# ZHANGKEON/DIS-YOLO

Measured on AMD Instinct MI355X. Metric: train images/sec @576x576 bf16, higher is better.
Workload: dtype bf16

## Files before the change

### dis-yolo_amd/csrc/conv_wgrad.hip

```cpp
#include "common.h"
#include "runtime.h"

namespace {

struct WgradParams {
  const bf16* x0;
  const bf16* x1;
  const bf16* dy;
  float* out;
  int B, H, W, C0, C1, Cin;
  int Ho, Wo, Cout, ldy;
  int ks, stride, pad_t, pad_l;
  int M, K;
  int steps_per_split, steps;
  int tilesK, tilesN;
  unsigned bytes0, bytes1, bytesy;
};

typedef __attribute__((address_space(3))) s16x4 lds_s16x4;
typedef int i32x4 __attribute__((ext_vector_type(4)));
constexpr unsigned OOB = 0x80000000u;

__device__ __forceinline__ int swz_u(int row, int u, int units) {
  const int h = (row & 3) | (((row >> 3) & 1) << 2);
// ... 461 lines not shown
  }

  float* slab = p.out + (size_t)bsplit * 9 * p.Cin * p.Cout;
  wait_vmcnt<0>();
  __syncthreads();
  constexpr int WTN = CO_T / 2;
  constexpr int ROWP = WTN * 4 + 16;
  constexpr int CPR4 = WTN / 4;
  char* sw = smem + wave * (16 * ROWP);
#pragma unroll
  for (int i = 0; i < TPW; ++i) {
    if (NW == 8 && i >= ntaps) continue;
    const int tap = tap0 + i;
#pragma unroll
    for (int j = 0; j < NJ; ++j)
#pragma unroll
      for (int r = 0; r < 4; ++r) *reinterpret_cast<float*>(sw + (g * 4 + r) * ROWP + (j * 16 + li) * 4) = acc[i][j][r];
    __builtin_amdgcn_fence(__ATOMIC_RELEASE, "wavefront");
    __builtin_amdgcn_wave_barrier();
    __builtin_amdgcn_fence(__ATOMIC_ACQUIRE, "wavefront");
#pragma unroll
    for (int it = 0; it < (16 * CPR4) / 64; ++it) {
      const int idx = it * 64 + lane;
      const int row = idx / CPR4, c4 = idx % CPR4;
      const int kk = tap * p.Cin + ci0 + u * 16 + row, n = co0 + ch * WTN + c4 * 4;
      if (n < p.Cout && !(p.debug & 1))
        *reinterpret_cast<float4*>(slab + (size_t)kk * p.Cout + n) = *reinterpret_cast<const float4*>(sw + row * ROWP + c4 * 16);
    }
    __builtin_amdgcn_fence(__ATOMIC_RELEASE, "wavefront");
    __builtin_amdgcn_wave_barrier();
  }
}

__global__ __launch_bounds__(256) void slab_reduce_kernel(const float* slabs, float* out, int64_t n, int splits) {
  __shared__ float sh[4][64];
  const int o = threadIdx.x & 63, g = threadIdx.x >> 6;
  const int64_t i = (int64_t)blockIdx.x * 64 + o;
  float a0 = 0.f, a1 = 0.f, a2 = 0.f, a3 = 0.f;
  if (i < n) {
    int k = g;
    for (; k + 12 < splits; k += 16) {
      a0 += slabs[(size_t)k * n + i];
      a1 += slabs[(size_t)(k + 4) * n + i];
      a2 += slabs[(size_t)(k + 8) * n + i];
      a3 += slabs[(size_t)(k + 12) * n + i];
    }
    for (; k < splits; k += 4) a0 += slabs[(size_t)k * n + i];
  }
  sh[g][o] = (a0 + a1) + (a2 + a3);
  __syncthreads();
  if (g == 0 && i < n) out[i] = (sh[0][o] + sh[1][o]) + (sh[2][o] + sh[3][o]);
}

__global__ __launch_bounds__(1024) void conv_first_wgrad_kernel(const float* img, const bf16* dy, float* slabs, int B,
                                                                int H, int W, int Cout, int px_per_block) {
  const int M = B * H * W;
  const int o = threadIdx.x;
  const int nout = 27 * Cout;
  if (o >= nout) return;
  const int k = o / Cout, co = o - k * Cout;
  const int tap = k / 3, ci = k - tap * 3;
  const int kh = tap / 3, kw = tap - kh * 3;
  const int m0 = blockIdx.x * px_per_block;
  int m1 = m0 + px_per_block;
  if (m1 > M) m1 = M;
  float acc = 0.f;
  for (int m = m0; m < m1; ++m) {
    const int b = m / (H * W);
    const int rem = m - b * H * W;
    const int y = rem / W, x = rem - y * W;
    const int iy = y + kh - 1, ix = x + kw - 1;
    if ((unsigned)iy < (unsigned)H && (unsigned)ix < (unsigned)W)
      acc += img[((size_t)(b * H + iy) * W + ix) * 3 + ci] * (float)dy[(size_t)m * Cout + co];
  }
  slabs[(size_t)blockIdx.x * nout + o] = acc;
}

constexpr int F1_ROWB = 272;
constexpr int F1_IMGB = 27 * F1_ROWB + 80;
constexpr int F1_STB = F1_IMGB + 8192;

__global__ __launch_bounds__(512) void conv_first_wgrad_mfma_kernel(const float* img, const bf16* dy, float* slabs, int B,
                                                                   int H, int W, int units_x, int nunits, unsigned bytesy) {
  extern __shared__ __attribute__((aligned(16))) char smem[];
// ... 273 lines not shown
  if (plan3(d, opts, &q3)) {
    Wg3Params p;
    p.x = (const bf16*)d->x0;
    p.dy = (const bf16*)dy;
    p.B = d->B; p.H = d->H; p.W = d->W; p.Cin = d->C0; p.Cout = d->Cout; p.ldy = dy_ld;
    p.Ho = d->Ho; p.Wo = d->Wo;
    p.P = d->Wo + 1; p.Hp = d->Ho + 1; p.frame = p.Hp * p.P;
    p.kbias = q3.s2 ? 0 : ceil_div((q3.leadB + 1) * 64, p.frame);
    p.a64 = 64 / p.P; p.r64 = 64 % p.P;
    p.chunks = q3.chunks; p.chunks_per_split = q3.cps;
    p.tilesCi = q3.tilesCi; p.tilesCo = q3.tilesCo; p.tiles = q3.tilesCi * q3.tilesCo;
    p.leadA = q3.leadA; p.leadB = q3.leadB;
    p.bytesx = (unsigned)((size_t)d->B * d->H * d->W * d->C0 * 2);
    p.bytesy = (unsigned)((size_t)d->B * d->Ho * d->Wo * dy_ld * 2);
    p.out = q3.splits == 1 ? dw : (float*)workspace;
    p.debug = 0;
    hipStream_t s = (hipStream_t)stream;
    if (opts & DISYOLO_WGRAD_REDUCE_ONLY) goto reduce3;
    if (q3.s2) {
      launch3_s2(p, q3, s);
    } else if (q3.co_t == 128) {
      if (q3.R == 8) launch3<128, 8>(p, q3, s);
      else if (q3.R == 16) launch3<128, 16>(p, q3, s);
      else launch3<128, 32>(p, q3, s);
    } else {
      if (q3.R == 8) launch3<64, 8>(p, q3, s);
      else if (q3.R == 16) launch3<64, 16>(p, q3, s);
      else launch3<64, 32>(p, q3, s);
    }
    DY_CHECK_LAUNCH();
  reduce3:
    if (q3.splits > 1 && !(opts & DISYOLO_WGRAD_PARTIAL_ONLY)) {
      const int64_t n = (int64_t)9 * p.Cin * p.Cout;
      hipLaunchKernelGGL(slab_reduce_kernel, dim3(ceil_div(n, 64)), dim3(256), 0, s, (const float*)workspace, dw, n,
                         q3.splits);
      DY_CHECK_LAUNCH();
    }
    return DISYOLO_OK;
  }
  WgradParams p;
  p.x0 = (const bf16*)d->x0;
  p.x1 = (const bf16*)d->x1;
  p.dy = (const bf16*)dy;
  p.B = d->B; p.H = d->H; p.W = d->W; p.C0 = d->C0; p.C1 = d->C1; p.Cin = d->C0 + d->C1;
  p.Ho = d->Ho; p.Wo = d->Wo; p.Cout = d->Cout; p.ldy = dy_ld;
  p.ks = d->ksize; p.stride = d->stride; p.pad_t = d->pad_t; p.pad_l = d->pad_l;
  p.M = d->B * d->Ho * d->Wo;
  p.K = d->ksize * d->ksize * p.Cin;
  p.bytes0 = (unsigned)((size_t)d->B * d->H * d->W * d->C0 * 2);
  p.bytes1 = (unsigned)((size_t)d->B * (d->H / 2) * (d->W / 2) * d->C1 * 2);
  p.bytesy = (unsigned)((size_t)p.M * dy_ld * 2);
  int bn, splits;
  plan(d, &bn, &splits, &p.steps_per_split, &p.steps);
  p.out = splits == 1 ? dw : (float*)workspace;
  hipStream_t s = (hipStream_t)stream;
  p.tilesK = ceil_div(p.K, 128);
  p.tilesN = ceil_div(p.Cout, bn);
  dim3 grid(p.tilesK * p.tilesN * splits);
  const int sto = (opts & DISYOLO_WGRAD_STAGES_MASK) >> 4;
  const int st = sto ? sto + 1 : 3;
  if (opts & DISYOLO_WGRAD_REDUCE_ONLY) goto reduce1;
#define DY_WG(BNV, YB)                                                                                   \
  if (st == 2) hipLaunchKernelGGL((conv_wgrad_kernel<BNV, 2>), grid, dim3(256), 2 * (8192 + YB), s, p);      \
  else if (st == 3) hipLaunchKernelGGL((conv_wgrad_kernel<BNV, 3>), grid, dim3(256), 3 * (8192 + YB), s, p); \
  else hipLaunchKernelGGL((conv_wgrad_kernel<BNV, 4>), grid, dim3(256), 4 * (8192 + YB), s, p);
  if (bn == 128) { DY_WG(128, 8192) }
  else if (bn == 64) { DY_WG(64, 4096) }
  else { DY_WG(32, 4096) }
#undef DY_WG
  DY_CHECK_LAUNCH();
reduce1:
  if (splits > 1 && !(opts & DISYOLO_WGRAD_PARTIAL_ONLY)) {
    const int64_t n = (int64_t)p.K * p.Cout;
    hipLaunchKernelGGL(slab_reduce_kernel, dim3(ceil_div(n, 64)), dim3(256), 0, s, (const float*)workspace, dw, n,
                       splits);
    DY_CHECK_LAUNCH();
  }
  return DISYOLO_OK;
}

static int first_wgrad_blocks(int B, int H, int W) {
  const int64_t pairs = ((int64_t)B * H * ceil_div(W, 128) + 1) / 2;
  return (int)(pairs < 512 ? pairs : 512);
}

extern "C" size_t disyolo_conv_first_wgrad_workspace(int B, int H, int W, int Cout) {
  const int64_t M = (int64_t)B * H * W;
  const int blocks = ceil_div(M, 1024);
  const size_t direct = (size_t)blocks * 27 * Cout * sizeof(float);
  const size_t mfma = (size_t)first_wgrad_blocks(B, H, W) * 27 * 32 * sizeof(float);
  return direct > mfma ? direct : mfma;
}

extern "C" int disyolo_conv_first_wgrad(const float* images, const void* dy, float* dw, int B, int H, int W, int Cout,
                                        void* workspace, size_t workspace_bytes, void* stream) {
  DY_REQUIRE(images && dy && dw && B > 0 && H > 0 && W > 0 && Cout > 0 && 27 * Cout <= 1024, "first_wgrad: bad args");
  if (!workspace || workspace_bytes < disyolo_conv_first_wgrad_workspace(B, H, W, Cout)) {
    disyolo_set_error("first_wgrad: workspace too small");
    return DISYOLO_E_WORKSPACE;
  }
  DY_RECORD_OR_RUN([=](void* s) { return disyolo_conv_first_wgrad(images, dy, dw, B, H, W, Cout, workspace, workspace_bytes, s); });
  const int64_t M = (int64_t)B * H * W;
  hipStream_t s = (hipStream_t)stream;
  const int64_t n = 27 * Cout;
  if (Cout == 32 && M * 64 < (1LL << 31)) {
    const int units_x = ceil_div(W, 128);
    const int nunits = B * H * units_x;
    const int blocks = first_wgrad_blocks(B, H, W);
    hipLaunchKernelGGL(conv_first_wgrad_mfma_kernel, dim3(blocks), dim3(512), 4 * F1_STB, s, images, (const bf16*)dy,
                       (float*)workspace, B, H, W, units_x, nunits, (unsigned)(M * 64));
    DY_CHECK_LAUNCH();
    hipLaunchKernelGGL(slab_reduce_kernel, dim3(ceil_div(n, 64)), dim3(256), 0, s, (const float*)workspace, dw, n, blocks);
    DY_CHECK_LAUNCH();
    return DISYOLO_OK;
  }
  const int blocks = ceil_div(M, 1024);
  hipLaunchKernelGGL(conv_first_wgrad_kernel, dim3(blocks), dim3(1024), 0, s, images, (const bf16*)dy,
                     (float*)workspace, B, H, W, Cout, 1024);
  DY_CHECK_LAUNCH();
  hipLaunchKernelGGL(slab_reduce_kernel, dim3(ceil_div(n, 64)), dim3(256), 0, s, (const float*)workspace, dw, n,
                     blocks);
  DY_CHECK_LAUNCH();
  return DISYOLO_OK;
}
```

### dis-yolo_amd/lib.py

```python
from __future__ import annotations

import ctypes as C
import os
from typing import Optional

import numpy as np
import torch

_HERE = os.path.dirname(os.path.abspath(__file__))
LIB_PATH = os.environ.get("DISYOLO_LIB", os.path.join(_HERE, "libdisyolo_hip.so"))

GRAD_LD = 32
ROI_MAX = 16
ROI_W = 12
K_MAPS = (3, 5, 7)
MASK_STRIDES = (1, 2, 4)


def roi_w(k: int) -> int:
    return 2 * (k + 1) + 4


def block32_post(k: int) -> int:
    return {3: 1, 5: 2, 7: 3}[k]
# ... 29 lines not shown
_SIGS = {
    "disyolo_version": (C.c_int, []),
    "disyolo_last_error": (C.c_char_p, []),
    "disyolo_conv_desc_size": (C.c_size_t, []),
    "disyolo_find_contours": (C.c_int, [C.c_void_p, C.c_int, C.c_int, C.c_void_p, C.c_int64, C.c_void_p, C.c_void_p, C.c_int,
                                        C.POINTER(C.c_int), C.POINTER(C.c_int64)]),
    "disyolo_conv2d_stats_rows": (C.c_int, [C.POINTER(ConvDesc)]),
    "disyolo_conv2d_bn_bwd_stats_ok": (C.c_int, [C.POINTER(ConvDesc)]),
    "disyolo_conv2d_bn_fused_ok": (C.c_int, [C.POINTER(ConvDesc)]),
    "disyolo_cluster_sync_words": (C.c_int, [C.c_int]),
    "disyolo_cluster_sync_error": (C.c_int, [C.c_void_p, C.c_int]),
    "disyolo_conv2d_fwd": (C.c_int, [C.POINTER(ConvDesc), C.c_void_p]),
    "disyolo_conv2d_tile": (C.c_int, [C.POINTER(ConvDesc)] + [C.POINTER(C.c_int)] * 4),
    "disyolo_conv_first_fwd": (C.c_int, [C.c_void_p] * 5 + [C.c_int] * 4 + [C.c_float, C.c_void_p]),
    "disyolo_conv12_fused_ok": (C.c_int, [C.c_int] * 3),
    "disyolo_conv12_fused_fwd": (C.c_int, [C.c_void_p] * 8 + [C.c_int] * 3 + [C.c_float, C.c_void_p]),
    "disyolo_block32_fused_ok": (C.c_int, [C.c_int] * 6),
    "disyolo_block64_fused_ok": (C.c_int, [C.c_int] * 4),
    "disyolo_pack_quad": (C.c_int, [C.c_void_p, C.c_void_p, C.c_int, C.c_int, C.c_void_p]),
    "disyolo_dgrad_s2_quad_ok": (C.c_int, [C.c_int] * 5),
    "disyolo_dgrad_s2_quad": (C.c_int, [C.c_void_p] * 4 + [C.c_int] * 5 + [C.c_void_p]),
    "disyolo_block64_fused_fwd": (C.c_int, [C.c_void_p] * 8 + [C.c_int] * 4 + [C.c_float, C.c_void_p]),
    "disyolo_block32_fused_fwd": (C.c_int, [C.c_void_p, C.c_void_p, C.c_int, C.c_int] + [C.c_void_p] * 6 + [C.c_int] +
                                  [C.c_void_p] * 3 + [C.c_int] * 3 + [C.c_float, C.c_void_p]),
    "disyolo_conv2d_wgrad_workspace": (C.c_size_t, [C.POINTER(ConvDesc), C.c_int]),
    "disyolo_conv2d_wgrad": (C.c_int, [C.POINTER(ConvDesc), C.c_void_p, C.c_int, C.c_void_p, C.c_void_p,
                                       C.c_size_t, C.c_int, C.c_void_p]),
    "disyolo_conv2d_fp8_fwd": (C.c_int, [C.POINTER(ConvDesc), C.c_void_p, C.c_void_p, C.c_void_p, C.c_void_p, C.c_float,
                                         C.c_void_p, C.c_float, C.c_void_p, C.c_void_p]),
    "disyolo_conv_first_fwd_fp8": (C.c_int, [C.c_void_p] * 5 + [C.c_float] + [C.c_int] * 4 + [C.c_float, C.c_void_p]),
    "disyolo_quant_fp8": (C.c_int, [C.c_void_p, C.c_int, C.c_void_p, C.c_int64, C.c_float, C.c_void_p]),
    "disyolo_dequant_fp8": (C.c_int, [C.c_void_p, C.c_void_p, C.c_int64, C.c_float, C.c_void_p]),
    "disyolo_pack_weights_fp8": (C.c_int, [C.c_void_p, C.c_void_p] + [C.c_int] * 3 + [C.c_float, C.c_void_p]),
    "disyolo_conv2d_wgrad_plan": (C.c_int, [C.POINTER(ConvDesc), C.c_int] + [C.POINTER(C.c_int)] * 4),
    "disyolo_conv_first_wgrad_workspace": (C.c_size_t, [C.c_int] * 4),
    "disyolo_conv_first_wgrad": (C.c_int, [C.c_void_p] * 3 + [C.c_int] * 4 + [C.c_void_p, C.c_size_t, C.c_void_p]),
    "disyolo_image_pad8": (C.c_int, [C.c_void_p, C.c_void_p, C.c_int64, C.c_void_p]),
    "disyolo_copy2d_f32": (C.c_int, [C.c_void_p, C.c_void_p] + [C.c_int] * 4 + [C.c_void_p]),
    "disyolo_pack_weights": (C.c_int, [C.c_void_p] * 3 + [C.c_int] * 4 + [C.c_void_p]),
    "disyolo_pack_table_bytes": (C.c_size_t, [C.c_int]),
    "disyolo_pack_table_build": (C.c_int, [C.c_void_p, C.c_int, C.c_void_p, C.POINTER(C.c_int)]),
    "disyolo_pack_all": (C.c_int, [C.c_void_p, C.c_int, C.c_int, C.c_void_p]),
    "disyolo_bn_finalize": (C.c_int, [C.c_void_p, C.c_int, C.c_int, C.c_int64] + [C.c_void_p] * 4 +
                            [C.c_float, C.c_float] + [C.c_void_p] * 5),
    "disyolo_colstats_rows": (C.c_int, [C.c_int64, C.c_int]),
    "disyolo_colstats": (C.c_int, [C.c_void_p, C.c_void_p, C.c_int64, C.c_int, C.c_void_p]),
    "disyolo_bn_fold": (C.c_int, [C.c_void_p] * 4 + [C.c_float] + [C.c_void_p] * 2 + [C.c_int, C.c_void_p]),
    "disyolo_bn_act_fwd": (C.c_int, [C.c_void_p] * 5 + [C.c_int64, C.c_int, C.c_float, C.c_void_p]),
    "disyolo_bn_act_bwd_workspace": (C.c_size_t, [C.c_int64, C.c_int]),
    "disyolo_bn_act_bwd_partials_workspace": (C.c_size_t, [C.c_int]),
    "disyolo_bn_act_bwd_partials": (C.c_int, [C.c_void_p] * 9 + [C.c_int64, C.c_int, C.c_float, C.c_void_p, C.c_int,
                                              C.c_void_p, C.c_int, C.c_void_p, C.c_size_t, C.c_void_p]),
    "disyolo_bn_partial_sums": (C.c_int, [C.c_void_p, C.c_int, C.c_int, C.c_void_p, C.c_void_p]),
    "disyolo_bn_finalize_sums": (C.c_int, [C.c_void_p, C.c_int, C.c_int64] + [C.c_void_p] * 4 + [C.c_float, C.c_float] +
                                 [C.c_void_p] * 5),
    "disyolo_bn_bwd_reduce_rows": (C.c_int, [C.c_int64, C.c_int]),
    "disyolo_bn_bwd_reduce": (C.c_int, [C.c_void_p] * 6 + [C.c_int64, C.c_int, C.c_float, C.c_void_p, C.c_void_p, C.c_size_t,
                                        C.c_void_p]),
    "disyolo_bn_bwd_apply_sums": (C.c_int, [C.c_void_p] * 8 + [C.c_int64] + [C.c_void_p] * 3 + [C.c_int64, C.c_int, C.c_float,
                                            C.c_void_p, C.c_int, C.c_void_p, C.c_size_t, C.c_void_p]),
    "disyolo_bn_act_bwd": (C.c_int, [C.c_void_p] * 9 + [C.c_int64, C.c_int, C.c_float, C.c_void_p, C.c_int, C.c_void_p, C.c_size_t,
                                                       C.c_void_p]),
    "disyolo_upsample2x_bwd": (C.c_int, [C.c_void_p] * 2 + [C.c_int] * 7 + [C.c_void_p]),
    "disyolo_colsum_workspace": (C.c_size_t, [C.c_int64, C.c_int]),
    "disyolo_colsum": (C.c_int, [C.c_void_p, C.c_void_p, C.c_int64, C.c_int, C.c_int, C.c_void_p, C.c_size_t,
                                 C.c_void_p]),
# ... 102 lines not shown
    return None if t is None else t.data_ptr()


def _stream() -> int:
    return torch.cuda.current_stream().cuda_stream


def _need(t: torch.Tensor, dtype, name: str) -> None:
    if t.dtype != dtype or not t.is_cuda or not t.is_contiguous():
        raise DisyoloError("%s must be a contiguous CUDA tensor of %s (got %s on %s)" % (name, dtype, t.dtype, t.device))


def _need_shape(t: torch.Tensor, shape, name: str) -> None:
    if tuple(t.shape) != tuple(shape):
        raise DisyoloError("%s must have shape %s (got %s)" % (name, tuple(shape), tuple(t.shape)))


class Workspace:

    def __init__(self, device):
        self.device = device
        self.buf = torch.empty(1 << 20, dtype=torch.uint8, device=device)
        self.frozen = False

    def get(self, nbytes: int) -> torch.Tensor:
        if self.buf.numel() < nbytes:
            if self.frozen:
                raise DisyoloError("workspace of %d bytes is frozen by a recorded command list; %d requested"
                                   % (self.buf.numel(), nbytes))
            self.buf = torch.empty(int(nbytes * 1.25) + 256, dtype=torch.uint8, device=self.device)
        return self.buf


class CmdList:

    def __init__(self):
        self.h = load().disyolo_cmdlist_create()
        self.keep = []
        self._side = None
        self._lanes = {}

    def __del__(self):
        try:
            if self.h:
                if torch.cuda.is_available() and (self._side is not None or self._lanes):
                    for st in [self._side] + list(self._lanes.values()):
                        if st is not None:
                            torch.cuda.current_stream(st.device).wait_stream(st)
                load().disyolo_cmdlist_destroy(self.h)
        except Exception:
            pass

    def __enter__(self):
        global TIMER
        if TIMER is not None:
            raise DisyoloError("cannot record a command list while the kernel timer is active")
        _check(load().disyolo_cmdlist_begin(self.h), "cmdlist_begin")
        global CURRENT_LANE
        CURRENT_LANE = 0
        return self

    def __exit__(self, *exc):
        _check(load().disyolo_cmdlist_end(), "cmdlist_end")
        global CURRENT_LANE
        CURRENT_LANE = 0
        return False
# ... 359 lines not shown
        TIMER.run("block64_kernel", 2.0 * M * (64 * 128 + 128 * 576), fn, float(M * 512))
        return
    fn()


def conv_first_fwd(images, w_hwio, scale, shift, y, alpha=0.1) -> None:
    _need(images, torch.float32, "images")
    _need(y, torch.bfloat16, "y")
    B, H, W, _ = images.shape
    _check(load().disyolo_conv_first_fwd(_p(images), _p(w_hwio), _p(scale), _p(shift), _p(y), B, H, W, y.shape[-1],
                                         alpha, _stream()), "conv_first_fwd")


WGRAD_IM2COL, WGRAD_PARTIAL_ONLY, WGRAD_REDUCE_ONLY = 1, 2, 4


def wgrad_stages(n: int) -> int:
    if not 2 <= int(n) <= 4:
        raise DisyoloError("wgrad_stages: 2..4 pipeline stages (got %r)" % (n,))
    return (int(n) - 1) << 4


def conv2d_wgrad_workspace(d: ConvDesc, opts: int = 0) -> int:
    return load().disyolo_conv2d_wgrad_workspace(C.byref(d), opts)


def conv2d_wgrad(d: ConvDesc, dy, dy_ld: int, dw, ws: Workspace, opts: int = 0) -> None:
    need = conv2d_wgrad_workspace(d, opts)
    buf = ws.get(need)

    def call(o):
        _check(load().disyolo_conv2d_wgrad(C.byref(d), _p(dy), dy_ld, _p(dw), _p(buf), buf.numel(), o, _stream()),
               "conv2d_wgrad")
    if TIMER is not None and not (opts & (WGRAD_PARTIAL_ONLY | WGRAD_REDUCE_ONLY)):
        kind, tn, ring, splits = conv2d_wgrad_plan(d, opts)
        name = ("conv_wgrad3x3_kernel<%d,%d,3,4,0>" % (tn, ring)) if kind == 1 else ("conv_wgrad_kernel<%d,3>" % tn)
        if kind == 1 and d.stride == 2:
            name = "conv_wgrad3x3_kernel<64,8,3,4,1>"
        TIMER.run(name, conv_flops(d), lambda: call(opts | WGRAD_PARTIAL_ONLY))
        if splits > 1:
            TIMER.run("slab_reduce_kernel", 0.0, lambda: call(opts | WGRAD_REDUCE_ONLY))
        return
    call(opts)


def conv2d_wgrad_plan(d: ConvDesc, opts: int = 0):
    v = [C.c_int(0) for _ in range(4)]
    _check(load().disyolo_conv2d_wgrad_plan(C.byref(d), opts, *[C.byref(x) for x in v]), "conv2d_wgrad_plan")
    return tuple(x.value for x in v)


def conv_first_wgrad(images, dy, dw, ws: Workspace) -> None:
    B, H, W, _ = images.shape
    cout = dy.shape[-1]
    need = load().disyolo_conv_first_wgrad_workspace(B, H, W, cout)
    buf = ws.get(need)
    _check(load().disyolo_conv_first_wgrad(_p(images), _p(dy), _p(dw), B, H, W, cout, _p(buf), buf.numel(), _stream()),
           "conv_first_wgrad")


def copy2d_f32(src, dst, rows, cols, src_ld, dst_ld) -> None:
    _check(load().disyolo_copy2d_f32(_p(src), _p(dst), rows, cols, src_ld, dst_ld, _stream()), "copy2d_f32")


def pack_weights(w_hwio, w_fwd, w_dgrad, ksize, cin, cout, cout_pad=0) -> None:
    _check(load().disyolo_pack_weights(_p(w_hwio), _p(w_fwd), _p(w_dgrad), ksize, cin, cout, max(cout_pad, cout),
                                       _stream()), "pack_weights")


class PackJob(C.Structure):
    _fields_ = [("w_hwio", C.c_void_p), ("w_fwd", C.c_void_p), ("w_dgrad", C.c_void_p),
                ("ksize", C.c_int32), ("Cin", C.c_int32), ("Cout", C.c_int32), ("cout_pad", C.c_int32)]


class PackTable:

    def __init__(self, jobs, device):
        n = len(jobs)
        arr = (PackJob * n)()
        for i, (w, wf, wd, k, cin, cout, pad) in enumerate(jobs):
            arr[i] = PackJob(_p(w), _p(wf), _p(wd), k, cin, cout, pad)
        nbytes = load().disyolo_pack_table_bytes(n)
# ... 397 lines not shown
```

### dis-yolo_amd/net.py

```python
from __future__ import annotations

from typing import Dict, List, Optional, Sequence, Tuple

import math
import json
import contextlib
import os
import sys
import numpy as np
import torch

from . import config as cfg
from . import lib as L

BF16 = torch.bfloat16
F32 = torch.float32

WGRAD_GROUP = 3
OPT_CHUNK_ELEMS = 8_000_000
PIPE_LANE = 2


class Layer:
    __slots__ = ("idx", "cin", "cout", "k", "stride", "kind", "src", "src_up", "shortcut", "lock", "H", "W", "Ho",
# ... 366 lines not shown
            g1 = S // 32
            self.labels = [torch.zeros(B, g, g, 3, 5 + self.num_class, dtype=F32, device=dev)
                           for g in (4 * g1, 2 * g1, g1)]
            self.true_boxes = torch.zeros(B, G, 5, dtype=F32, device=dev)
            self.true_masks = torch.zeros(B, G, S, S, dtype=torch.uint8, device=dev)
            self.perm_det = torch.arange(cfg.MAX_DETECTION, dtype=torch.int32, device=dev).repeat(B, 1).contiguous()
            self.perm_gt = torch.arange(G, dtype=torch.int32, device=dev).repeat(B, 1).contiguous()
            self.rois = torch.zeros(B, L.ROI_MAX, L.roi_w(self.k), dtype=torch.int32, device=dev)
            self.roi_count = torch.zeros(B, dtype=torch.int32, device=dev)
            self._in_sets = None
            if self.pair:
                names = ("labels", "true_boxes", "true_masks", "perm_det", "perm_gt", "clip_window")
                first = {n: getattr(self, n) for n in names}
                second = {n: ([t.clone() for t in v] if isinstance(v, list) else v.clone()) for n, v in first.items()}
                self._in_sets = [first, second]
            self.losses = torch.zeros(8, dtype=F32, device=dev)
            self.mask_loss = torch.zeros(1, dtype=F32, device=dev)
            self.reg_loss = torch.zeros(1, dtype=F32, device=dev)
            self.loss_ring = torch.zeros(self.LOSS_RING, dtype=F32, device=dev)
            tmax = 0
            for l in self.layers:
                if l.src_up is not None and l.wdg is not None:
                    tmax = max(tmax, B * l.H * l.W * self.by_idx[l.src_up].cout)
            self.up_tmp = torch.zeros(max(tmax, 1), dtype=BF16, device=dev)
            need = 1 << 20
            for l in self.layers:
                if l.wgrad_desc is not None:
                    need = max(need, L.conv2d_wgrad_workspace(l.wgrad_desc))
                if l.dx is not None and l.kind != "lin":
                    need = max(need, L.load().disyolo_bn_act_bwd_workspace(B * l.Ho * l.Wo, l.cout))
            if not l1.lock:
                need = max(need, L.load().disyolo_conv_first_wgrad_workspace(B, S, S, l1.cout))
            self.ws.get(int(need))
            self.ws_aux.get(int(need))
        self.ws_det.get(int(max(L.load().disyolo_detect_workspace(B, S, self.num_class), 1 << 20)))
        self._build_dgrad_descs()
        self.refresh_weights()

    FP8_FROM = int(os.environ.get("DISYOLO_FP8_FROM", "10"))
    FP8_UPTO = 52
    FP8_DUAL = (4, 9, 26, 43, 52)

    def _fp8_layers(self):
        return [l for l in self.layers if self.FP8_FROM <= l.idx <= self.FP8_UPTO and (l.lock or not self.training)]

    def _plan_fp8(self) -> None:
        dev = self.device
        ls = self._fp8_layers()
        if [l.idx for l in ls] != list(range(self.FP8_FROM, self.FP8_UPTO + 1)) or not all(
                l.lock or not self.training for l in self.layers[:self.FP8_UPTO]):
            raise L.DisyoloError("dtype='fp8' needs conv1-52 in inference mode (stage 1 training, or training=False)")
        if self.FP8_FROM <= 1 and any(1 in (l.src, l.src_up) for l in self.layers if l.idx > 2):
            raise L.DisyoloError("dtype='fp8' with DISYOLO_FP8_FROM=1 and mask_stride=1: conv83 needs act1 in bf16")
        self._fp8_entry = self.by_idx[self.FP8_FROM - 1] if self.FP8_FROM > 1 else None
        if self._fp8_entry is not None:
            q = self._fp8_entry
            q.act8 = torch.zeros(self.B, q.Ho, q.Wo, q.cout, dtype=torch.uint8, device=dev)
            q.s_out = 1.0
        for l in ls:
            l.act8 = torch.zeros(self.B, l.Ho, l.Wo, l.cout, dtype=torch.uint8, device=dev)
            l.escale = torch.zeros(l.cout, dtype=F32, device=dev)
            l.dual16 = l.idx in self.FP8_DUAL
            l.s_out, l.s_w = 1.0, 1.0
            if l.idx > 1:
                l.w8 = torch.zeros(l.cout, l.k * l.k * l.cin, dtype=torch.uint8, device=dev)
                l.desc8 = L.make_conv_desc(self.by_idx[l.src].act8, l.w8, l.act8, l.k, l.stride, leaky=True, alpha=cfg.ALPHA)

# ... 681 lines not shown
                                 bn_bwd=(tgt.raw, tgt.scale, tgt.shift, tgt.mean, tgt.rstd, tgt.bwd_part, cfg.ALPHA),
                                 bn_bwd_fused=dict(dgamma=tgt.dgamma, dbeta=tgt.dbeta, sync=tgt.csync_bwd))
            tgt.fused_bwd = True
        L.conv2d_fwd(d)

    def check_cluster_sync(self) -> None:
        for l in self.layers:
            for name, buf in (("forward", l.csync), ("backward", l.csync_bwd)):
                if buf is not None:
                    code = L.cluster_sync_error(buf, l.cout)
                    if code:
                        raise L.DisyoloError("conv%d: the in-launch batch-norm exchange (%s) timed out (code %#x): another launch of "
                                             "that kind was running on this device, or the grid was not resident; the results of "
                                             "this run are wrong (DISYOLO_BN_INKERNEL=0 switches the feature off)" % (l.idx, name, code))

    def _shortcut_feeds_grad(self, tgt: Layer) -> bool:
        return tgt.shortcut is not None and self.by_idx[tgt.shortcut].grad is not None

    def _final_writers(self, visit) -> Dict[int, Tuple[int, str]]:
        last: Dict[int, Tuple[int, str]] = {}
        for l in visit:
            if l.lock:
                continue
            if l.kind != "lin" and l.shortcut is not None and self.by_idx[l.shortcut].grad is not None:
                last[l.shortcut] = (l.idx, "add")
            for mode, tgt, _ in l.dgrad_descs:
                last[tgt.idx] = (l.idx, mode)
        return last

    def backward_order(self) -> List[Layer]:
        heads = [self.by_idx[i] for i in (75, 74, 67, 66, 59, 58)]
        return heads + [l for l in reversed(self.layers) if l.idx not in self.HEAD_LAYERS]

    def backward(self, on_layer_done=None, sweep: bool = False) -> None:
        B = self.B
        for l in self.layers:
            l.grad_set = False
        visit = self.backward_order()
        order = [l for l in visit if not l.lock]
        final_of = {} if self.sync_bn else self._final_writers(visit)
        for l in self.layers:
            l.bwd_part_rows = 0
            l.fused_bwd = False
        inl = self.dp is not None and self.dp.inlist
        overlap_opt = sweep and (self.dp is None or inl) and self.n_params > 0
        if overlap_opt:
            if self.opt_chunks is None:
                self._plan_opt_chunks()
            self._opt_swept = set()
            self._opt_done = [set() for _ in self.opt_chunks]
        pending: list = []

        def flush():
            if not pending:
                return
            side_g = pending[0][4]
            mark = L.lane_mark(0) if side_g else None
            waited = False
            for (pl, pdx, pld, pM, pside) in pending:
                if pside:
                    if not waited:
                        L.lane_wait(mark, 1)
                        waited = True
                    L.set_lane(1)
                wsl = self.ws_aux if pside else self.ws
                if pl.kind == "lin":
                    L.colsum(pl.dx, pl.dbias, pM, pl.cout_pad, pl.cout, wsl)
                if pl.idx == 1:
                    L.conv_first_wgrad(self.images, pl.dx, pl.dw, wsl)
                else:
                    L.conv2d_wgrad(pl.wgrad_desc, pdx, pld, pl.dw, wsl)
                if pside:
                    L.set_lane(0)
                if self._overlap_rec:
                    for src, reader in self._xstep_reader.items():
                        if reader == pl.idx and self._xstep_slot[src] in self._xstep_waits.values():
                            L.lane_mark_slot(1 if pside else 0, self._xstep_slot[src])
                if overlap_opt and pside:
                    ci = self._opt_chunk_of[pl.idx]
                    self._opt_done[ci].add(pl.idx)
                    if self._opt_done[ci] == self.opt_chunks[ci]["members"]:
                        if inl:
                            L.lane_wait(L.lane_mark(1), L.COMM_LANE)
                            L.set_lane(L.COMM_LANE)
                            ch = self.opt_chunks[ci]
                            self.dp.exchange_inlist(ci, ch["off"], ch["cnt"])
                            self._sweep_chunk(ci, 1.0 / self.dp.world_size)
                            L.set_lane(0)
                        else:
                            L.set_lane(1)
                            self._sweep_chunk(ci, 1.0)
                            L.set_lane(0)
                if on_layer_done is not None:
                    on_layer_done(pl)
            pending.clear()

        for l in visit:
            pos = order.index(l) if not l.lock else -1
            if l.idx == self.score_layer and getattr(self, "_mask_loss_pending", False):
                L.lane_wait(self._mask_mark, 0)
                self._mask_loss_pending = False
            if l.lock:
                continue
            M = B * l.Ho * l.Wo
            if l.kind == "lin":
                dx, ld = l.dx, l.cout_pad
# ... 454 lines not shown
```

### include/disyolo.h

```cpp
#ifndef DISYOLO_H
#define DISYOLO_H

#include <stddef.h>
#include <stdint.h>

#ifdef __cplusplus
extern "C" {
#endif

#define DISYOLO_OK 0
#define DISYOLO_E_ARG (-1)
#define DISYOLO_E_WORKSPACE (-2)
#define DISYOLO_E_HIP (-3)

#define DISYOLO_GRAD_LD 32
#define DISYOLO_ROI_MAX 16
#define DISYOLO_ROI_W 12
#define DISYOLO_ROI_W_K(k) (2 * ((k) + 1) + 4)

int disyolo_version(void);
const char* disyolo_last_error(void);

enum {
  DISYOLO_CONV_LEAKY = 1,
// ... 59 lines not shown
int disyolo_conv_first_fwd(const float* images, const float* w_hwio, const float* scale,
                           const float* shift, void* y_bf16, int B, int H, int W, int Cout,
                           float alpha, void* stream);

int disyolo_conv12_fused_ok(int B, int H, int W);
int disyolo_conv12_fused_fwd(const float* images, const float* w1_hwio, const float* scale1, const float* shift1,
                             const void* w2_packed, const float* scale2, const float* shift2, void* y_bf16, int B, int H,
                             int W, float alpha, void* stream);

int disyolo_block32_fused_ok(int B, int H, int W, int C0, int C1, int post);
int disyolo_block32_fused_fwd(const void* x0, const void* x1, int C0, int C1, const void* wA, const float* scaleA,
                              const float* shiftA, const void* wB, const float* scaleB, const float* shiftB, int post,
                              const void* wC, const float* biasC, void* y, int B, int H, int W, float alpha, void* stream);

int disyolo_block64_fused_ok(int B, int H, int W, int C0);
int disyolo_block64_fused_fwd(const void* x, const void* wA, const float* scaleA, const float* shiftA, const void* wB,
                              const float* scaleB, const float* shiftB, void* y, int B, int H, int W, int C0, float alpha,
                              void* stream);

int disyolo_pack_quad(const float* w_hwio, void* wq, int C, int Cdy, void* stream);
int disyolo_dgrad_s2_quad_ok(int B, int Hdy, int Wdy, int Cdy, int C);
int disyolo_dgrad_s2_quad(const void* dy, const void* wq, void* dx, const void* residual, int B, int Hdy, int Wdy, int Cdy,
                          int C, void* stream);

enum {
  DISYOLO_WGRAD_IM2COL = 1,
  DISYOLO_WGRAD_PARTIAL_ONLY = 2,
  DISYOLO_WGRAD_REDUCE_ONLY = 4,
  DISYOLO_WGRAD_STAGES_MASK = 0x30
};
size_t disyolo_conv2d_wgrad_workspace(const disyolo_conv_desc* d, int opts);
int disyolo_conv2d_wgrad(const disyolo_conv_desc* d, const void* dy, int dy_ld, float* dw,
                         void* workspace, size_t workspace_bytes, int opts, void* stream);
int disyolo_conv2d_fp8_fwd(const disyolo_conv_desc* d, const void* w_fp8, const float* escale,
                           const float* eshift, const void* residual_fp8, float residual_scale,
                           void* y_fp8, float out_scale, void* y_bf16, void* stream);
int disyolo_conv_first_fwd_fp8(const float* images, const float* w_hwio, const float* scale, const float* shift,
                               void* y_fp8, float out_scale, int B, int H, int W, int Cout, float alpha,
                               void* stream);
int disyolo_quant_fp8(const void* x, int x_is_f32, void* y_fp8, int64_t n, float scale, void* stream);
int disyolo_dequant_fp8(const void* x_fp8, float* y, int64_t n, float scale, void* stream);
int disyolo_pack_weights_fp8(const float* w_hwio, void* w_fp8, int ksize, int Cin, int Cout,
                             float scale, void* stream);

int disyolo_conv2d_wgrad_plan(const disyolo_conv_desc* d, int opts, int* kind, int* tile_n, int* ring, int* splits);
size_t disyolo_conv_first_wgrad_workspace(int B, int H, int W, int Cout);
int disyolo_conv_first_wgrad(const float* images, const void* dy, float* dw, int B, int H, int W,
                             int Cout, void* workspace, size_t workspace_bytes, void* stream);

int disyolo_image_pad8(const float* images, void* out_bf16, int64_t pixels, void* stream);
int disyolo_copy2d_f32(const float* src, float* dst, int rows, int cols, int src_ld, int dst_ld,
                       void* stream);

int disyolo_pack_weights(const float* w_hwio, void* w_fwd, void* w_dgrad, int ksize, int Cin,
                         int Cout, int cout_pad, void* stream);

typedef struct disyolo_pack_job {
  const float* w_hwio;
  void* w_fwd;
  void* w_dgrad;
  int32_t ksize, Cin, Cout, cout_pad;
} disyolo_pack_job;
size_t disyolo_pack_table_bytes(int njobs);
int disyolo_pack_table_build(const disyolo_pack_job* jobs, int njobs, void* host_table, int* total_blocks);
int disyolo_pack_all(const void* device_table, int njobs, int total_blocks, void* stream);

// ... 164 lines not shown
```

Baseline: 2157.

## Batch split-K weight-gradient reductions across layers into one vectorized slab-sum kernel

Replaces the per-layer scalar slab reduce with a float4-vectorized, grid-strided slab_sum kernel that can process a table of up to 8 jobs. In backward, the pending wgrad layers of a group now write partials into disjoint workspace regions and run PARTIAL_ONLY, and one batched reduce launch then sums all their slabs. The aim is fewer kernel launches and wider memory accesses for the split-K reduction. In exchange the auxiliary workspace grows to hold several layers' slabs, a device job table is cached per group, and lane synchronization moves to cover the whole group.

```diff
diff --git a/dis-yolo_amd/csrc/conv_wgrad.hip b/dis-yolo_amd/csrc/conv_wgrad.hip
--- a/dis-yolo_amd/csrc/conv_wgrad.hip
+++ b/dis-yolo_amd/csrc/conv_wgrad.hip
@@ -517,24 +517,112 @@
   }
 }
 
-__global__ __launch_bounds__(256) void slab_reduce_kernel(const float* slabs, float* out, int64_t n, int splits) {
-  __shared__ float sh[4][64];
+struct SlabPlan {
+  const float* slabs;
+  float* out;
+  int64_t n;
+  int64_t n4;
+  int64_t ns;
+  int64_t unit0;
+  int64_t vunits;
+  int splits;
+  int head;
+  int out16;
+};
+constexpr int SLAB_MAX_JOBS = DISYOLO_SLAB_MAX_JOBS;
+constexpr int SLAB_MAX_BLOCKS = 1024;
+
+__device__ __host__ inline int64_t slab_plan(const disyolo_slab_job& j, SlabPlan* q) {
+  q->slabs = j.slabs; q->out = j.out; q->n = j.n; q->splits = j.splits;
+  q->head = 0; q->n4 = 0; q->out16 = 0;
+  if (j.n >= 4 && (j.n & 3) == 0) {
+    q->head = (int)(((16u - (unsigned)((size_t)j.slabs & 15u)) & 15u) >> 2);
+    q->n4 = (j.n - q->head) >> 2;
+    q->out16 = ((size_t)(j.out + q->head) & 15u) == 0;
+  }
+  q->ns = j.n - 4 * q->n4;
+  q->vunits = (q->n4 + 63) >> 6;
+  return q->vunits + ((q->ns + 63) >> 6);
+}
+
+__device__ inline float4 add4(const float4 a, const float4 b) { return make_float4(a.x + b.x, a.y + b.y, a.z + b.z, a.w + b.w); }
+
+__global__ __launch_bounds__(256) void slab_sum_kernel(const disyolo_slab_job* jobs, int njobs, disyolo_slab_job one) {
+  __shared__ float4 sh[4][64];
+  __shared__ SlabPlan plans[SLAB_MAX_JOBS];
+  __shared__ int64_t total_sh;
+  if (threadIdx.x == 0) {
+    int64_t u = 0;
+    for (int j = 0; j < njobs; ++j) {
+      plans[j].unit0 = u;
+      u += slab_plan(jobs ? jobs[j] : one, &plans[j]);
+    }
+    total_sh = u;
+  }
+  __syncthreads();
+  const int64_t total = total_sh;
   const int o = threadIdx.x & 63, g = threadIdx.x >> 6;
-  const int64_t i = (int64_t)blockIdx.x * 64 + o;
-  float a0 = 0.f, a1 = 0.f, a2 = 0.f, a3 = 0.f;
-  if (i < n) {
-    int k = g;
-    for (; k + 12 < splits; k += 16) {
-      a0 += slabs[(size_t)k * n + i];
-      a1 += slabs[(size_t)(k + 4) * n + i];
-      a2 += slabs[(size_t)(k + 8) * n + i];
-      a3 += slabs[(size_t)(k + 12) * n + i];
-    }
-    for (; k < splits; k += 4) a0 += slabs[(size_t)k * n + i];
-  }
-  sh[g][o] = (a0 + a1) + (a2 + a3);
-  __syncthreads();
-  if (g == 0 && i < n) out[i] = (sh[0][o] + sh[1][o]) + (sh[2][o] + sh[3][o]);
+  for (int64_t u = blockIdx.x; u < total; u += gridDim.x) {
+    int j = 0;
+    while (j + 1 < njobs && u >= plans[j + 1].unit0) ++j;
+    const SlabPlan& q = plans[j];
+    const int64_t lu = u - q.unit0, n = q.n;
+    const int splits = q.splits;
+    if (lu < q.vunits) {
+      const int64_t c = lu * 64 + o;
+      float4 a0 = make_float4(0.f, 0.f, 0.f, 0.f), a1 = a0, a2 = a0, a3 = a0;
+      if (c < q.n4) {
+        const float* col = q.slabs + q.head + 4 * c;
+        int k = g;
+        for (; k + 12 < splits; k += 16) {
+          a0 = add4(a0, *reinterpret_cast<const float4*>(col + (size_t)k * n));
+          a1 = add4(a1, *reinterpret_cast<const float4*>(col + (size_t)(k + 4) * n));
+          a2 = add4(a2, *reinterpret_cast<const float4*>(col + (size_t)(k + 8) * n));
+          a3 = add4(a3, *reinterpret_cast<const float4*>(col + (size_t)(k + 12) * n));
+        }
+        for (; k < splits; k += 4) a0 = add4(a0, *reinterpret_cast<const float4*>(col + (size_t)k * n));
+      }
+      sh[g][o] = add4(add4(a0, a1), add4(a2, a3));
+      __syncthreads();
+      if (g == 0 && c < q.n4) {
+        const float4 r = add4(add4(sh[0][o], sh[1][o]), add4(sh[2][o], sh[3][o]));
+        float* dst = q.out + q.head + 4 * c;
+        if (q.out16) {
+          *reinterpret_cast<float4*>(dst) = r;
+        } else {
+          dst[0] = r.x; dst[1] = r.y; dst[2] = r.z; dst[3] = r.w;
+        }
+      }
+    } else {
+      const int64_t e = (lu - q.vunits) * 64 + o;
+      const int64_t i = e < q.head ? e : e + 4 * q.n4;
+      float a0 = 0.f, a1 = 0.f, a2 = 0.f, a3 = 0.f;
+      if (e < q.ns) {
+        const float* col = q.slabs + i;
+        int k = g;
+        for (; k + 12 < splits; k += 16) {
+          a0 += col[(size_t)k * n];
+          a1 += col[(size_t)(k + 4) * n];
+          a2 += col[(size_t)(k + 8) * n];
+          a3 += col[(size_t)(k + 12) * n];
+        }
+        for (; k < splits; k += 4) a0 += col[(size_t)k * n];
+      }
+      sh[g][o].x = (a0 + a1) + (a2 + a3);
+      __syncthreads();
+      if (g == 0 && e < q.ns) q.out[i] = (sh[0][o].x + sh[1][o].x) + (sh[2][o].x + sh[3][o].x);
+    }
+    __syncthreads();
+  }
+}
+
+static int slab_grid(int64_t units) { return (int)(units < 1 ? 1 : (units < SLAB_MAX_BLOCKS ? units : SLAB_MAX_BLOCKS)); }
+
+static void slab_sum_launch(const float* slabs, float* out, int64_t n, int splits, hipStream_t s) {
+  const disyolo_slab_job one = {slabs, out, n, splits, 0};
+  SlabPlan q;
+  hipLaunchKernelGGL(slab_sum_kernel, dim3(slab_grid(slab_plan(one, &q))), dim3(256), 0, s, (const disyolo_slab_job*)nullptr, 1,
+                     one);
 }
 
 __global__ __launch_bounds__(1024) void conv_first_wgrad_kernel(const float* img, const bf16* dy, float* slabs, int B,
@@ -874,8 +962,7 @@
   reduce3:
     if (q3.splits > 1 && !(opts & DISYOLO_WGRAD_PARTIAL_ONLY)) {
       const int64_t n = (int64_t)9 * p.Cin * p.Cout;
-      hipLaunchKernelGGL(slab_reduce_kernel, dim3(ceil_div(n, 64)), dim3(256), 0, s, (const float*)workspace, dw, n,
-                         q3.splits);
+      slab_sum_launch((const float*)workspace, dw, n, q3.splits, s);
       DY_CHECK_LAUNCH();
     }
     return DISYOLO_OK;
@@ -914,10 +1001,27 @@
 reduce1:
   if (splits > 1 && !(opts & DISYOLO_WGRAD_PARTIAL_ONLY)) {
     const int64_t n = (int64_t)p.K * p.Cout;
-    hipLaunchKernelGGL(slab_reduce_kernel, dim3(ceil_div(n, 64)), dim3(256), 0, s, (const float*)workspace, dw, n,
-                       splits);
+    slab_sum_launch((const float*)workspace, dw, n, splits, s);
     DY_CHECK_LAUNCH();
   }
+  return DISYOLO_OK;
+}
+
+extern "C" int disyolo_slab_reduce(const float* slabs, float* out, int64_t n, int splits, void* stream) {
+  DY_REQUIRE(slabs && out && n > 0 && splits > 0, "slab_reduce: bad args");
+  DY_RECORD_OR_RUN([=](void* s) { return disyolo_slab_reduce(slabs, out, n, splits, s); });
+  slab_sum_launch(slabs, out, n, splits, (hipStream_t)stream);
+  DY_CHECK_LAUNCH();
+  return DISYOLO_OK;
+}
+
+extern "C" int disyolo_slab_reduce_batched(const disyolo_slab_job* device_jobs, int njobs, int64_t total_n, void* stream) {
+  DY_REQUIRE(device_jobs && njobs > 0 && njobs <= SLAB_MAX_JOBS && total_n > 0, "slab_reduce_batched: bad args");
+  DY_RECORD_OR_RUN([=](void* s) { return disyolo_slab_reduce_batched(device_jobs, njobs, total_n, s); });
+  const disyolo_slab_job none = {nullptr, nullptr, 0, 0, 0};
+  hipLaunchKernelGGL(slab_sum_kernel, dim3(slab_grid((total_n + 255) / 256 + 2 * (int64_t)njobs)), dim3(256), 0, (hipStream_t)stream,
+                     device_jobs, njobs, none);
+  DY_CHECK_LAUNCH();
   return DISYOLO_OK;
 }
 
@@ -952,7 +1056,7 @@
     hipLaunchKernelGGL(conv_first_wgrad_mfma_kernel, dim3(blocks), dim3(512), 4 * F1_STB, s, images, (const bf16*)dy,
                        (float*)workspace, B, H, W, units_x, nunits, (unsigned)(M * 64));
     DY_CHECK_LAUNCH();
-    hipLaunchKernelGGL(slab_reduce_kernel, dim3(ceil_div(n, 64)), dim3(256), 0, s, (const float*)workspace, dw, n, blocks);
+    slab_sum_launch((const float*)workspace, dw, n, blocks, s);
     DY_CHECK_LAUNCH();
     return DISYOLO_OK;
   }
@@ -960,8 +1064,7 @@
   hipLaunchKernelGGL(conv_first_wgrad_kernel, dim3(blocks), dim3(1024), 0, s, images, (const bf16*)dy,
                      (float*)workspace, B, H, W, Cout, 1024);
   DY_CHECK_LAUNCH();
-  hipLaunchKernelGGL(slab_reduce_kernel, dim3(ceil_div(n, 64)), dim3(256), 0, s, (const float*)workspace, dw, n,
-                     blocks);
+  slab_sum_launch((const float*)workspace, dw, n, blocks, s);
   DY_CHECK_LAUNCH();
   return DISYOLO_OK;
 }
diff --git a/dis-yolo_amd/lib.py b/dis-yolo_amd/lib.py
--- a/dis-yolo_amd/lib.py
+++ b/dis-yolo_amd/lib.py
@@ -85,6 +85,8 @@
     "disyolo_quant_fp8": (C.c_int, [C.c_void_p, C.c_int, C.c_void_p, C.c_int64, C.c_float, C.c_void_p]),
     "disyolo_dequant_fp8": (C.c_int, [C.c_void_p, C.c_void_p, C.c_int64, C.c_float, C.c_void_p]),
     "disyolo_pack_weights_fp8": (C.c_int, [C.c_void_p, C.c_void_p] + [C.c_int] * 3 + [C.c_float, C.c_void_p]),
+    "disyolo_slab_reduce": (C.c_int, [C.c_void_p, C.c_void_p, C.c_int64, C.c_int, C.c_void_p]),
+    "disyolo_slab_reduce_batched": (C.c_int, [C.c_void_p, C.c_int, C.c_int64, C.c_void_p]),
     "disyolo_conv2d_wgrad_plan": (C.c_int, [C.POINTER(ConvDesc), C.c_int] + [C.POINTER(C.c_int)] * 4),
     "disyolo_conv_first_wgrad_workspace": (C.c_size_t, [C.c_int] * 4),
     "disyolo_conv_first_wgrad": (C.c_int, [C.c_void_p] * 3 + [C.c_int] * 4 + [C.c_void_p, C.c_size_t, C.c_void_p]),
@@ -253,6 +255,17 @@
         return self.buf
 
 
+class WorkspaceRegion:
+
+    def __init__(self, buf: torch.Tensor, off: int, nbytes: int):
+        self.buf = buf[off:off + nbytes]
+
+    def get(self, nbytes: int) -> torch.Tensor:
+        if self.buf.numel() < nbytes:
+            raise DisyoloError("workspace region of %d bytes; %d requested" % (self.buf.numel(), nbytes))
+        return self.buf
+
+
 class CmdList:
 
     def __init__(self):
@@ -678,14 +691,15 @@
     def call(o):
         _check(load().disyolo_conv2d_wgrad(C.byref(d), _p(dy), dy_ld, _p(dw), _p(buf), buf.numel(), o, _stream()),
                "conv2d_wgrad")
-    if TIMER is not None and not (opts & (WGRAD_PARTIAL_ONLY | WGRAD_REDUCE_ONLY)):
+    if TIMER is not None and not (opts & WGRAD_REDUCE_ONLY):
         kind, tn, ring, splits = conv2d_wgrad_plan(d, opts)
         name = ("conv_wgrad3x3_kernel<%d,%d,3,4,0>" % (tn, ring)) if kind == 1 else ("conv_wgrad_kernel<%d,3>" % tn)
         if kind == 1 and d.stride == 2:
             name = "conv_wgrad3x3_kernel<64,8,3,4,1>"
         TIMER.run(name, conv_flops(d), lambda: call(opts | WGRAD_PARTIAL_ONLY))
-        if splits > 1:
-            TIMER.run("slab_reduce_kernel", 0.0, lambda: call(opts | WGRAD_REDUCE_ONLY))
+        if splits > 1 and not (opts & WGRAD_PARTIAL_ONLY):
+            K = d.ksize * d.ksize * (d.C0 + d.C1)
+            TIMER.run("slab_sum_kernel", 0.0, lambda: call(opts | WGRAD_REDUCE_ONLY), float((splits + 1) * K * d.Cout * 4))
         return
     call(opts)
 
@@ -694,6 +708,49 @@
     v = [C.c_int(0) for _ in range(4)]
     _check(load().disyolo_conv2d_wgrad_plan(C.byref(d), opts, *[C.byref(x) for x in v]), "conv2d_wgrad_plan")
     return tuple(x.value for x in v)
+
+
+def slab_reduce(slabs, out, n: int, splits: int) -> None:
+    _need(slabs, torch.float32, "slabs")
+    _need(out, torch.float32, "out")
+    if slabs.numel() < n * splits or out.numel() < n:
+        raise DisyoloError("slab_reduce: %d x %d elements do not fit the tensors given" % (splits, n))
+    _check(load().disyolo_slab_reduce(_p(slabs), _p(out), n, splits, _stream()), "slab_reduce")
+
+
+SLAB_MAX_JOBS = 8
+
+
+class SlabJob(C.Structure):
+    _fields_ = [("slabs", C.c_void_p), ("out", C.c_void_p), ("n", C.c_int64), ("splits", C.c_int32), ("reserved", C.c_int32)]
+
+
+class SlabTable:
+
+    def __init__(self, jobs, device):
+        n = len(jobs)
+        if not 1 <= n <= SLAB_MAX_JOBS:
+            raise DisyoloError("SlabTable: 1..%d jobs (got %d)" % (SLAB_MAX_JOBS, n))
+        arr = (SlabJob * n)()
+        for i, (slabs, out, cnt, splits) in enumerate(jobs):
+            _need(slabs, torch.float32, "slabs")
+            _need(out, torch.float32, "out")
+            if cnt < 1 or splits < 1 or slabs.numel() < cnt * splits or out.numel() < cnt:
+                raise DisyoloError("SlabTable: job %d: %d x %d elements do not fit the tensors given" % (i, splits, cnt))
+            arr[i] = SlabJob(_p(slabs), _p(out), cnt, splits, 0)
+        self.n = n
+        self.total = sum(j[2] for j in jobs)
+        self.bytes = float(sum((j[3] + 1) * j[2] * 4 for j in jobs))
+        self.dev = torch.frombuffer(bytearray(bytes(arr)), dtype=torch.uint8).to(device)
+        self.keep = jobs
+
+    def run(self) -> None:
+        fn = lambda: _check(load().disyolo_slab_reduce_batched(_p(self.dev), self.n, self.total, _stream()),
+                            "slab_reduce_batched")
+        if TIMER is not None:
+            TIMER.run("slab_sum_kernel", 0.0, fn, self.bytes)
+            return
+        fn()
 
 
 def conv_first_wgrad(images, dy, dw, ws: Workspace) -> None:
diff --git a/dis-yolo_amd/net.py b/dis-yolo_amd/net.py
--- a/dis-yolo_amd/net.py
+++ b/dis-yolo_amd/net.py
@@ -422,7 +422,11 @@
             if not l1.lock:
                 need = max(need, L.load().disyolo_conv_first_wgrad_workspace(B, S, S, l1.cout))
             self.ws.get(int(need))
+            sizes = [self._wgrad_region_bytes(l) for l in self.backward_order() if not l.lock]
+            for i in range(len(sizes)):
+                need = max(need, sum(sizes[i:i + WGRAD_GROUP]))
             self.ws_aux.get(int(need))
+            self._slab_groups = {}
         self.ws_det.get(int(max(L.load().disyolo_detect_workspace(B, S, self.num_class), 1 << 20)))
         self._build_dgrad_descs()
         self.refresh_weights()
@@ -1170,6 +1174,38 @@
         heads = [self.by_idx[i] for i in (75, 74, 67, 66, 59, 58)]
         return heads + [l for l in reversed(self.layers) if l.idx not in self.HEAD_LAYERS]
 
+    def _wgrad_region_bytes(self, l) -> int:
+        if l.idx == 1:
+            need = L.load().disyolo_conv_first_wgrad_workspace(self.B, self.S, self.S, l.cout)
+        else:
+            need = L.conv2d_wgrad_workspace(l.wgrad_desc)
+        if l.kind == "lin":
+            need = max(need, L.load().disyolo_colsum_workspace(self.B * l.Ho * l.Wo, l.cout_pad))
+        return (int(need) + 255) & ~255
+
+    def _slab_group(self, group, ws):
+        sizes = [self._wgrad_region_bytes(l) for l in group]
+        buf = ws.get(sum(sizes))
+        key = (tuple(l.idx for l in group), buf.data_ptr())
+        hit = self._slab_groups.get(key)
+        if hit is not None:
+            return hit
+        regions, jobs, off = [], [], 0
+        for l, sz in zip(group, sizes):
+            regions.append(L.WorkspaceRegion(buf, off, sz))
+            off += sz
+            if l.idx != 1:
+                d = l.wgrad_desc
+                splits = L.conv2d_wgrad_plan(d)[3]
+                n = d.ksize * d.ksize * (d.C0 + d.C1) * d.Cout
+                if l.dw.numel() != n:
+                    raise L.DisyoloError("layer %d: weight gradient of %d elements, descriptor says %d" % (l.idx, l.dw.numel(), n))
+                if splits > 1:
+                    jobs.append((regions[-1].buf.view(F32), l.dw, n, splits))
+        table = L.SlabTable(jobs, self.device) if jobs else None
+        self._slab_groups[key] = (regions, table)
+        return regions, table
+
     def backward(self, on_layer_done=None, sweep: bool = False) -> None:
         B = self.B
         for l in self.layers:
@@ -1194,22 +1230,24 @@
                 return
             side_g = pending[0][4]
             mark = L.lane_mark(0) if side_g else None
-            waited = False
-            for (pl, pdx, pld, pM, pside) in pending:
-                if pside:
-                    if not waited:
-                        L.lane_wait(mark, 1)
-                        waited = True
-                    L.set_lane(1)
-                wsl = self.ws_aux if pside else self.ws
+            wsg = self.ws_aux if side_g else self.ws
+            regions, table = self._slab_group([p[0] for p in pending], wsg) if len(pending) > 1 else (None, None)
+            if side_g:
+                L.lane_wait(mark, 1)
+                L.set_lane(1)
+            for gi, (pl, pdx, pld, pM, pside) in enumerate(pending):
+                wsl = regions[gi] if regions is not None else wsg
                 if pl.kind == "lin":
                     L.colsum(pl.dx, pl.dbias, pM, pl.cout_pad, pl.cout, wsl)
                 if pl.idx == 1:
                     L.conv_first_wgrad(self.images, pl.dx, pl.dw, wsl)
                 else:
-                    L.conv2d_wgrad(pl.wgrad_desc, pdx, pld, pl.dw, wsl)
-                if pside:
-                    L.set_lane(0)
+                    L.conv2d_wgrad(pl.wgrad_desc, pdx, pld, pl.dw, wsl, L.WGRAD_PARTIAL_ONLY if regions is not None else 0)
+            if table is not None:
+                table.run()
+            if side_g:
+                L.set_lane(0)
+            for (pl, pdx, pld, pM, pside) in pending:
                 if self._overlap_rec:
                     for src, reader in self._xstep_reader.items():
                         if reader == pl.idx and self._xstep_slot[src] in self._xstep_waits.values():
diff --git a/include/disyolo.h b/include/disyolo.h
--- a/include/disyolo.h
+++ b/include/disyolo.h
@@ -115,6 +115,16 @@
 size_t disyolo_conv2d_wgrad_workspace(const disyolo_conv_desc* d, int opts);
 int disyolo_conv2d_wgrad(const disyolo_conv_desc* d, const void* dy, int dy_ld, float* dw,
                          void* workspace, size_t workspace_bytes, int opts, void* stream);
+#define DISYOLO_SLAB_MAX_JOBS 8
+typedef struct disyolo_slab_job {
+  const float* slabs;
+  float* out;
+  int64_t n;
+  int32_t splits;
+  int32_t reserved;
+} disyolo_slab_job;
+int disyolo_slab_reduce(const float* slabs, float* out, int64_t n, int splits, void* stream);
+int disyolo_slab_reduce_batched(const disyolo_slab_job* device_jobs, int njobs, int64_t total_n, void* stream);
 int disyolo_conv2d_fp8_fwd(const disyolo_conv_desc* d, const void* w_fp8, const float* escale,
                            const float* eshift, const void* residual_fp8, float residual_scale,
                            void* y_fp8, float out_scale, void* y_bf16, void* stream);
```

Result: no change. 2148, median of 3 (-0.4%).
